# Ryan21wy/HSIMAE

Measured on AMD Instinct MI355X. Metric: HSI patches/sec (9x9x96, mask 75%) pretrain fwd+bwd, higher is better.
Workload: dtype bf16; 1 GPU; HSIMAE-Base pretrain fwd+bwd, 9x9x96 cubes, per-GPU batch 4096, mask 0.75, bf16 MFMA operands / fp32 accumulate + residual; per_gpu_batch=4096, global_batch=4096, parallelism=dp1

## Files before the change

hsimae_amd/build.py:

```python
from __future__ import annotations

import os
import subprocess
import sys
from concurrent.futures import ThreadPoolExecutor

HERE = os.path.dirname(os.path.abspath(__file__))
CSRC = os.path.join(HERE, "csrc")
LIB = os.path.join(HERE, "libhsimae_hip.so")
UNITS = ["gemm", "attn", "attn_wide", "wgrad", "elem", "pack", "fused_dec", "fused_enc", "loader", "scene", "gwpca", "api"]
HIPCC = os.environ.get("HIPCC", "/opt/rocm/bin/hipcc")
BASE_FLAGS = ["--offload-arch=gfx950", "-O3", "-fPIC", "-std=c++17", "-Wno-unused-value", "-fvisibility=hidden"]
FLAGS = BASE_FLAGS + os.environ.get("HSIMAE_HIPCC_EXTRA", "").split()


def flags_hash(flags: list[str]) -> str:
    import hashlib
    return hashlib.sha256(" ".join(flags).encode()).hexdigest()[:16]


def unit_flags(unit: str, flags: list[str]) -> list[str]:
    if unit != "api":
        return list(flags)
    return list(flags) + [f"-DHS_BUILD_FLAGS_HASH=0x{flags_hash(flags)}ULL", f"-DHS_BUILD_DEFAULT_FLAGS={int(flags == BASE_FLAGS)}",
                          f"-DHS_KERNEL_SOURCE_HASH=0x{kernel_source_hash()}ULL"]


def kernel_source_hash() -> str:
    import hashlib
    h = hashlib.sha256()
    files = sorted(os.path.join(CSRC, f) for f in os.listdir(CSRC) if f.endswith((".hip", ".h", ".cpp")))
    files.append(os.path.join(HERE, "..", "include", "hsimae_hip.h"))
    for f in files:
# ... 76 lines not shown
```

hsimae_amd/csrc/api.hip:

```cpp
#include "common.h"
#include "kernels.h"
#include "plan.h"
#include <vector>
#include <algorithm>
#include <cstring>
#include <cstdlib>
#include <mutex>
#include <unordered_map>
#include <initializer_list>

using namespace hsplan;

namespace {

#define CK(expr) do { int _e = (expr); if (_e) return _e; } while (0)
#define CK0(expr) do { int _e0 = (expr); if (_e0) return _e0; } while (0)

inline hipStream_t S(void* s) { return reinterpret_cast<hipStream_t>(s); }
struct BlkP {
    const float *n1w, *n1b, *bqkv, *pb, *n2w, *n2b, *w1b, *w3b, *w2b;
    const hs_bf16 *qkv, *p, *w1, *w3, *w2, *qkvT, *pT, *w13T, *w2T;
    const float *qf, *kf, *vf, *pf, *w1f, *w3f;
    int prec;
    struct I8 { const uint8_t* w; const uint8_t* s; } qkv8, p8, w1_8, w3_8, w2_8, qkvT8, pT8, w13T8, w2T8;
// ... 10 lines not shown
    const uint8_t* base8 = reinterpret_cast<const uint8_t*>(fbase + WL.f32_elems);
    auto i8 = [&](const Img8& im) { BlkP::I8 r; r.w = base8 + im.w; r.s = base8 + im.s; return r; };
    b.prec = HSIMAE_PREC_BF16;
    b.qkv8 = i8(w.qkv8); b.p8 = i8(w.p8); b.w1_8 = i8(w.w1_8); b.w3_8 = i8(w.w3_8); b.w2_8 = i8(w.w2_8);
    b.qkvT8 = i8(w.qkvT8); b.pT8 = i8(w.pT8); b.w13T8 = i8(w.w13T8); b.w2T8 = i8(w.w2T8);
    return b;
}
enum : uint32_t {
    SC_FUSED_DEC = 1u << 0,
    SC_DEC_SPLIT = 1u << 1,
    SC_FP8_UNFUSED = 1u << 2,
    SC_FUSED_MLP = 1u << 3,
    SC_ATTN_BLOCK = 1u << 4,
    SC_ATTN_BLOCK256 = 1u << 5,
    SC_ATTN_BLOCK_BWD = 1u << 6,
    SC_PROJ_BWD = 1u << 7,
    SC_LNBWD = 1u << 8,
    SC_LNBWD_512 = 1u << 9,
    SC_RECOMPUTE = 1u << 10,
    SC_WGRAD_SLAB = 1u << 11,
    SC_DEC_SLAB = 1u << 12,
    SC_PLANAR = 1u << 13,
    SC_ATTN_BLOCK256_BWD = 1u << 14,
};
uint32_t sched_from_env() {
    auto off = [](const char* name) { const char* e = getenv(name); return e && e[0] == '0'; };
    auto one = [](const char* name) { const char* e = getenv(name); return e && e[0] == '1'; };
    uint32_t b = 0;
    if (!off("HSIMAE_FUSED_DEC")) b |= SC_FUSED_DEC;
    if (!off("HSIMAE_DEC_SPLIT")) b |= SC_DEC_SPLIT;
    if (one("HSIMAE_FP8_UNFUSED")) b |= SC_FP8_UNFUSED;
    if (!off("HSIMAE_FUSED_MLP")) b |= SC_FUSED_MLP;
    if (!off("HSIMAE_FUSED_ATTN_BLOCK")) b |= SC_ATTN_BLOCK;
    if (!off("HSIMAE_FUSED_ATTN_BLOCK256")) b |= SC_ATTN_BLOCK256;
    if (!off("HSIMAE_FUSED_ATTN_BLOCK_BWD")) b |= SC_ATTN_BLOCK_BWD;
    if (!off("HSIMAE_FUSED_PROJ_BWD")) b |= SC_PROJ_BWD;
    if (!off("HSIMAE_FUSED_LNBWD")) b |= SC_LNBWD;
    if (!off("HSIMAE_FUSED_LNBWD_512")) b |= SC_LNBWD_512;
    if (!off("HSIMAE_ATTN_BWD_RECOMPUTE")) b |= SC_RECOMPUTE;
    if (!off("HSIMAE_WGRAD_SLAB")) b |= SC_WGRAD_SLAB;
    if (!off("HSIMAE_DEC_SLAB")) b |= SC_DEC_SLAB;
    if (!off("HSIMAE_WGRAD_PLANAR")) b |= SC_PLANAR;
    if (!off("HSIMAE_FUSED_ATTN_BLOCK256_BWD")) b |= SC_ATTN_BLOCK256_BWD;
    return b;
}
struct SchedRec { uint32_t enc = 0, dec = 0; bool has_enc = false, has_dec = false; uint64_t gen = 0; };
std::mutex g_sched_mu;
std::unordered_map<const void*, SchedRec> g_sched;
uint64_t g_sched_gen = 0;
void record_sched(const void* ws, bool enc, bool dec, uint32_t bits) {
    std::lock_guard<std::mutex> lk(g_sched_mu);
    if (g_sched.size() > 4096 && g_sched.find(ws) == g_sched.end()) {
        std::vector<uint64_t> gens;
        gens.reserve(g_sched.size());
        for (auto& kv : g_sched) gens.push_back(kv.second.gen);
        std::nth_element(gens.begin(), gens.begin() + gens.size() / 2, gens.end());
        const uint64_t cut = gens[gens.size() / 2];
        for (auto it = g_sched.begin(); it != g_sched.end();) it = it->second.gen < cut ? g_sched.erase(it) : std::next(it);
    }
    SchedRec& r = g_sched[ws];
    r.gen = ++g_sched_gen;
    if (enc) {
        r.enc = bits; r.has_enc = true;
        if (!dec) r.has_dec = false;
    }
    if (dec) { r.dec = bits; r.has_dec = true; }
// ... 151 lines not shown
    return HSIMAE_OK;
}


static bool wide_ln_fused(int d, int dp, bool f8, uint32_t sc) {
    return (sc & SC_LNBWD) && dp == d && (d == 256 || (d == 512 && f8 && (sc & SC_LNBWD_512)));
}

int block_bwd(const BlkP& P, uint32_t sc, const BlkOff& o, float* grads, const float* x_in, const BlkBuf& b, int64_t M, int d,
              int heads, int h, int hp, int Ts, int nsamples, int mode, int len_l, float* G0, const Scr& w,
              float* dx_out, int accumulate, hipStream_t s, int concurrent = 1, const float* rs_a = nullptr,
              const float* rs_m = nullptr, int64_t* det_acc = nullptr) {
    float* G1 = w.G1;
    GemmParams p = gp();
    const int dp = rup(d, 32);
    LnBwdParams l; std::memset(&l, 0, sizeof(l));
    l.M = (int)M; l.d = d; l.ld = dp; l.det_base = grads; l.det_acc = det_acc;
    const bool f8 = P.prec == HSIMAE_PREC_FP8;
    const bool f8u = f8 && (sc & SC_FP8_UNFUSED);
    auto w8 = [&](GemmParams& q, const BlkP::I8& a) { if (f8) { q.prec = HSIMAE_PREC_FP8; q.W8 = a.w; q.S8 = a.s; } };
    const bool fmlp = !f8u && fused_mlp_enabled(d, h, sc);
    bool g1b_done = false;
    const int hp64 = rup(hp, 64);
    const bool planar = fmlp && (sc & SC_PLANAR) && M % 32 == 0 && (M + kPlanePadRows) * 2 * (int64_t)(hp64 + 256) * 2 < (1ll << 32);
    const int prow = planar ? (int)M + HS_PLANE_PAD_ROWS : 0;
    if (fmlp) {
        CK(hs_enc_mlp_bwd(b.x1, G0, G1, b.u2, w.dh13, b.g, w.g0b, w.g1b, (int)M, d, mlp_ptrs(P, h), grads + o.n2w,
                          grads + o.n2b, s, rs_m, rs_a, HsDet{grads, reinterpret_cast<long long*>(det_acc)}, prow));
    } else {
        p.A = G0; p.lda = dp; p.M = (int)M; p.N = hp; p.K = dp; p.n_valid = hp; p.W = P.w2T; p.out = w.dh13; p.ldo = 2 * hp;
        p.h13 = b.h13; p.ldh = 2 * hp; p.hoff = hp; p.a_rowscale = rs_m;
        w8(p, P.w2T8);
        CK(hs_gemm(p, A_F32, E_SWIGLU_BWD, s));
        p = gp();
        p.A = w.dh13; p.lda = 2 * hp; p.M = (int)M; p.N = dp; p.K = 2 * hp; p.n_valid = d; p.W = P.w13T;
        w8(p, P.w13T8);
        if (wide_ln_fused(d, dp, f8, sc)) {
            p.out = G1; p.ldo = dp; p.res = G0; p.ldr = dp; p.lnx = b.x1; p.gamma = P.n2w; p.accumulate = 0;
            p.dgamma = grads + o.n2w; p.dbeta = grads + o.n2b; p.det_base = grads; p.det_acc = det_acc;
            if (!rs_a) { p.u_out = w.g1b; p.ldu = dp; g1b_done = true; }
            CK(hs_gemm(p, A_BF16, E_LN_BWD, s));
        } else {
            p.out = w.du; p.ldo = dp;
            CK(hs_gemm(p, A_BF16, E_F32, s));
            l.du = w.du; l.x = b.x1; l.gamma = P.n2w; l.dres = G0; l.dx = G1; l.accumulate = 0;
            l.dgamma = grads + o.n2w; l.dbeta = grads + o.n2b;
            CK(hs_ln_bwd(l, s));
        }
        CK(hs_rows_to_bf16(G0, w.g0b, M, dp, rs_m, s));
        if (!g1b_done) CK(hs_rows_to_bf16(G1, w.g1b, M, dp, rs_a, s));
    }
    auto run_wgrad = [&]() -> int {
        WgradParams g; std::memset(&g, 0, sizeof(g));
        auto task = [&](int, const void* dO, int ldo, const hs_bf16* A, int lda, int N, int K, int64_t dW, int64_t db) {
            WgradTask& t = g.t[g.ntasks++];
            t.dO = dO; t.dO_f32 = 0; t.ldo = ldo; t.A = A; t.lda = lda; t.N = N; t.K = K; t.dW = grads + dW; t.ldw = K;
            t.db = grads + db; t.dO_rowscale = nullptr;
        };
        task(0, w.dqkv, 3 * dp, b.u, dp, d, d, o.qw, o.qb);
        task(1, w.dqkv + dp, 3 * dp, b.u, dp, d, d, o.kw, o.kb);
        task(2, w.dqkv + 2 * dp, 3 * dp, b.u, dp, d, d, o.vw, o.vb);
        task(3, w.g1b, dp, b.o, dp, d, d, o.pw, o.pb);
        if (planar) {
            task(4, w.dh13, hp64, b.u2, dp, h, d, o.w1w, o.w1b); g.t[g.ntasks - 1].dO_plane_rows = prow;
            task(5, w.dh13 + (int64_t)hp64 * prow, hp64, b.u2, dp, h, d, o.w3w, o.w3b); g.t[g.ntasks - 1].dO_plane_rows = prow;
        } else {
            task(4, w.dh13, 2 * hp, b.u2, dp, h, d, o.w1w, o.w1b);
            task(5, w.dh13 + hp, 2 * hp, b.u2, dp, h, d, o.w3w, o.w3b);
        }
#ifdef HS_ABL_DW2
        if (!fmlp)
#endif
        { task(6, w.g0b, dp, b.g, planar ? hp64 : hp, d, h, o.w2w, o.w2b); g.t[g.ntasks - 1].A_plane_rows = prow; }
        g.M = (int)M; g.det_base = grads; g.det_acc = det_acc;
        g.slab = (sc & SC_WGRAD_SLAB) ? w.slab : nullptr;
        int tiles = 0;
        for (int i = 0; i < g.ntasks; ++i) tiles += ((g.t[i].N + 127) / 128) * ((g.t[i].K + 127) / 128);
        g.msplit = wgrad_msplit(tiles, M, concurrent);
        return hs_wgrad(g, s);
    };
    AttnParams a; std::memset(&a, 0, sizeof(a));
    a.qkv = b.qkv; a.ld = 3 * dp; a.d = d; a.heads = heads; a.hd = d / heads; a.Ts = Ts; a.nsamples = nsamples;
    a.mode = mode; a.len_l = len_l; a.o = b.o; a.ldo = dp; a.lse = b.lse; a.dout = w.dob; a.lddo = dp; a.dqkv = w.dqkv; a.kv_off = dp;
    const bool fuse_pb = (sc & SC_PROJ_BWD) != 0;
    const bool fuse_ln = (sc & SC_LNBWD) != 0;
    const bool rc = attn_bwd_recompute(d, dp, heads, h, Ts, f8u, sc);
    const bool blk_bwd = rc || (fuse_pb && fuse_ln && fmlp && !f8u && d == 128 && dp == d && hs_attn_proj_fusable(a) &&
                                (sc & SC_ATTN_BLOCK_BWD) && hs_attn_block_bwd_fusable(d, heads, Ts));
    const bool blk256_bwd = !blk_bwd && !f8 && dp == d && (sc & SC_ATTN_BLOCK256_BWD) && (sc & SC_LNBWD) && (sc & SC_PROJ_BWD) &&
                            hs_attn_block256_bwd_fusable(d, heads, Ts, nsamples);
    if (blk256_bwd) {
        CK(hs_attn_block256_bwd(b.qkv, b.lse, w.g1b, G1, x_in, P.n1w, P.pT, P.qkvT, w.dqkv, dx_out, grads + o.n1w, grads + o.n1b, grads,
                                reinterpret_cast<long long*>(det_acc), Ts, nsamples, mode, len_l, accumulate, s));
        CK(run_wgrad());
        return HSIMAE_OK;
    }
    if (blk_bwd) {
        CK(hs_attn_block_bwd(rc ? nullptr : b.qkv, b.u, P.qkv, P.bqkv, b.o, b.lse, w.g1b, G1, x_in, P.n1w, P.pT, P.qkvT, w.dqkv, dx_out,
                             grads + o.n1w, grads + o.n1b, grads, reinterpret_cast<long long*>(det_acc), Ts, nsamples, mode, len_l,
                             accumulate, s));
// ... 41 lines not shown
    if (!io) return HSIMAE_ENULL;
    c.N = io->N; c.len_t = io->len_t; c.len_l = io->len_l;
    if (c.N <= 0 || c.len_t < 1 || c.len_t > c.g.T || c.len_l < 1 || c.len_l > 9) return HSIMAE_EDIMS;
    c.K = c.len_t * c.len_l;
    c.Me = (int64_t)c.N * c.K; c.Md = (int64_t)c.N * c.g.TL;
    if (c.Md * 96 >= (1ll << 31) || c.Me * 3 * c.g.Dp >= (1ll << 31)) return HSIMAE_EUNSUPPORTED;
    make_playout(c.g, c.L);
    make_wlayout(c.g, c.W);
    if (need_ws) {
        if (!io->workspace || !io->params || !io->wpk) return HSIMAE_ENULL;
        if (reinterpret_cast<uintptr_t>(io->workspace) % 256) return HSIMAE_EALIGN;
        carve(c.g, c.N, c.K, reinterpret_cast<char*>(io->workspace), c.w);
        if (c.w.bytes > io->workspace_bytes) return HSIMAE_EDIMS;
    }
    return HSIMAE_OK;
}

}

extern "C" unsigned hs_variant_bits_gemm();
extern "C" unsigned hs_variant_bits_attn();
extern "C" unsigned hs_variant_bits_attn_wide();
extern "C" unsigned hs_variant_bits_wgrad();
extern "C" unsigned hs_variant_bits_elem();
extern "C" unsigned hs_variant_bits_pack();
extern "C" unsigned hs_variant_bits_fused_dec();
extern "C" unsigned hs_variant_bits_fused_enc();
extern "C" unsigned hs_variant_bits_loader();
extern "C" unsigned hs_variant_bits_scene();
extern "C" unsigned hs_variant_bits_gwpca();
#ifndef HS_KERNEL_SOURCE_HASH
#define HS_KERNEL_SOURCE_HASH 0ULL
#endif
#ifndef HS_BUILD_FLAGS_HASH
#define HS_BUILD_FLAGS_HASH 0ULL
#endif
#ifndef HS_BUILD_DEFAULT_FLAGS
#define HS_BUILD_DEFAULT_FLAGS 0
#endif

extern "C" {

int hsimae_version(void) { return HSIMAE_VERSION; }

int hsimae_build_info(hsimae_build_info_t* out) {
    if (!out) return HSIMAE_ENULL;
    out->abi_version = HSIMAE_VERSION;
    out->variant_bits = hs_variant_bits() | hs_variant_bits_gemm() | hs_variant_bits_attn() | hs_variant_bits_attn_wide() | hs_variant_bits_wgrad() | hs_variant_bits_elem() | hs_variant_bits_pack() | hs_variant_bits_fused_dec() | hs_variant_bits_fused_enc() | hs_variant_bits_loader() | hs_variant_bits_scene() | hs_variant_bits_gwpca();
    out->kernel_source_hash = HS_KERNEL_SOURCE_HASH;
    out->flags_hash = HS_BUILD_FLAGS_HASH;
    out->default_flags = HS_BUILD_DEFAULT_FLAGS;
    out->reserved = 0;
    return HSIMAE_OK;
}
const char* hsimae_variant_name(int bit) {
    switch (bit) {
#define HS_X(b, name) case b: return #name;
        HS_VARIANT_TABLE(HS_X)
#undef HS_X
        default: return nullptr;
    }
}

int hsimae_two_streams_active(void) { return side().ok ? 1 : 0; }
int hsimae_effective_precision(const hsimae_config* cfg) {
    if (!cfg) return HSIMAE_ENULL;
    Geo g; CK(make_geo(cfg, g));
    return (g.prec == HSIMAE_PREC_FP8 && (g.D >= 512 || (sched_from_env() & SC_FP8_UNFUSED))) ? HSIMAE_PREC_FP8 : HSIMAE_PREC_BF16;
}

const char* hsimae_strerror(int code) {
// ... 528 lines not shown
```

hsimae_amd/csrc/fused_enc.hip:

```cpp
#include "common.h"
#include "kernels.h"
#include <cstdlib>

#ifdef HS_PHASE_TIMING
__device__ unsigned long long hs_phase_cycles_enc[32];
extern "C" __attribute__((visibility("default"))) int hsimae_debug_phases_enc(unsigned long long* out, int reset) {
    int rc = (int)hipMemcpyFromSymbol(out, HIP_SYMBOL(hs_phase_cycles_enc), sizeof(unsigned long long) * 32);
    if (reset) { unsigned long long z[32] = {0}; rc |= (int)hipMemcpyToSymbol(HIP_SYMBOL(hs_phase_cycles_enc), z, sizeof(z)); }
    return rc;
}
#define PH_DECL unsigned long long ph_t0 = __builtin_readcyclecounter(), ph_acc[8] = {0, 0, 0, 0, 0, 0, 0, 0};
#define PH(i) { const unsigned long long ph_t = __builtin_readcyclecounter(); ph_acc[i] += ph_t - ph_t0; ph_t0 = ph_t; }
#define PH_FLUSH(base) if (threadIdx.x == 0) { for (int i = 0; i < 8; ++i) atomicAdd(&hs_phase_cycles_enc[(base) + i], ph_acc[i]); }
#else
#define PH_DECL
#define PH(i)
#define PH_FLUSH(base)
#endif

#ifndef HS_NT_A
#define HS_NT_A 1
#endif
#ifndef HS_NT_B
#define HS_NT_B 0
// ... 335 lines not shown
    HsDet det;
    int plane_rows;
};

__device__ __forceinline__ __amdgpu_buffer_rsrc_t panel_rsrc(const void* base, long long rows, int row_bytes) {
    const long long b = rows > 0 ? (rows < 4096 ? rows : 4096) * row_bytes : 0;
    return __builtin_amdgcn_make_buffer_rsrc(const_cast<void*>(base), 0, (int)b, 0x00020000);
}
__device__ __forceinline__ void bld8(__amdgpu_buffer_rsrc_t r, unsigned bo, float* o) {
    const f32x4 a = __builtin_bit_cast(f32x4, __builtin_amdgcn_raw_buffer_load_b128(r, (int)bo, 0, 0));
    const f32x4 b = __builtin_bit_cast(f32x4, __builtin_amdgcn_raw_buffer_load_b128(r, (int)bo + 16, 0, 0));
    o[0] = a[0]; o[1] = a[1]; o[2] = a[2]; o[3] = a[3]; o[4] = b[0]; o[5] = b[1]; o[6] = b[2]; o[7] = b[3];
}
typedef __attribute__((ext_vector_type(4))) unsigned int u32q;
__device__ __forceinline__ void bst8f(__amdgpu_buffer_rsrc_t r, unsigned bo, const float* v) {
    __builtin_amdgcn_raw_buffer_store_b128(__builtin_bit_cast(u32q, f32x4{v[0], v[1], v[2], v[3]}), r, (int)bo, 0, 0);
    __builtin_amdgcn_raw_buffer_store_b128(__builtin_bit_cast(u32q, f32x4{v[4], v[5], v[6], v[7]}), r, (int)bo + 16, 0, 0);
}
__device__ __forceinline__ void bst8h(__amdgpu_buffer_rsrc_t r, unsigned bo, bf16x8 v, int aux) {
    if (aux) __builtin_amdgcn_raw_buffer_store_b128(__builtin_bit_cast(u32q, v), r, (int)bo, 0, 2);
    else __builtin_amdgcn_raw_buffer_store_b128(__builtin_bit_cast(u32q, v), r, (int)bo, 0, 0);
}

template <int D, int HPE, bool LATE_ST = false>
__global__ __launch_bounds__(NTH, (MG<D, HPE>::WPC)) void enc_mlp_bwd_kernel(EncMlpBwdArgs p) {
    using G = MG<D, HPE>;
    constexpr int R = G::R;
    constexpr int LU = G::LU, LC = G::LC, LX = G::LX, NCH = G::NCH, KSD = G::KSD, KSH = G::KSH, LPR = G::LPR;
    extern __shared__ __attribute__((aligned(16))) char smem[];
    bf16_t* U2 = reinterpret_cast<bf16_t*>(smem);
    bf16_t* DYb = U2 + R * LU;
    bf16_t* DH1 = DYb + R * LU;
    bf16_t* DH3 = DH1 + R * LC;
    bf16_t* Gc = DH3 + R * LC;
    float* XS = reinterpret_cast<float*>(G::XS_AT_DY ? reinterpret_cast<char*>(DYb) : smem);
    const G8 q = geo8<D>();
    const int row0 = blockIdx.x * R;
    const EncMlpW& w = p.w;
    const int nt_h = HPE / 16;
    const int c8 = (threadIdx.x % LPR) * 8;
    constexpr bool late_stores = LATE_ST;

    PH_DECL
    constexpr int MT4 = R / 16, NJO = D / 64;
    FrN<KSD, 1> f1, f3, f2;
    f1.template load<false>(w.w1, KSD, q.wave, 0, nt_h, q.lane);
    f3.template load<false>(w.w3, KSD, q.wave, 0, nt_h, q.lane);
// ... 94 lines not shown
                    f1.template load<false>(w.w1, KSD, (c + 1) * 4 + q.wave, 0, nt_h, q.lane);
                    f3.template load<false>(w.w3, KSD, (c + 1) * 4 + q.wave, 0, nt_h, q.lane);
                    f2.template load<false>(w.w2T, KSD, (c + 1) * 4 + q.wave, 0, nt_h, q.lane);
                } else {
                    f1.load(w.w1, KSD, (c + 1) * 4 + q.wave, 0, nt_h, q.lane);
                    f3.load(w.w3, KSD, (c + 1) * 4 + q.wave, 0, nt_h, q.lane);
                    f2.load(w.w2T, KSD, (c + 1) * 4 + q.wave, 0, nt_h, q.lane);
                }
            }
#endif
#pragma unroll
            for (int mt = 0; mt < MT4; ++mt) {
                f32x4 gv, d1, d3;
#pragma unroll
                for (int r = 0; r < 4; ++r) {
                    const float a1 = h1[mt][r], a3 = h3[mt][r], dv = dg[mt][r];
                    const float sg = __builtin_amdgcn_rcpf(1.f + __expf(-a1));
                    const float sl = a1 * sg;
                    gv[r] = sl * a3;
                    d1[r] = dv * a3 * sg * (1.f + a1 * (1.f - sg));
                    d3[r] = dv * sl;
                }
                const int o = ctile<LC>(mt, q);
                *reinterpret_cast<bf16x4*>(Gc + o) = cvt4(gv);
                *reinterpret_cast<bf16x4*>(DH1 + o) = cvt4(d1);
                *reinterpret_cast<bf16x4*>(DH3 + o) = cvt4(d3);
            }
        }
        lds_barrier();
        PH(1)
        constexpr bool LATE = D >= 256;
        FrN<2, NJO> wa;
        FrN<1, NJO> wb0, wb1;
#ifdef HS_ABL_WSTREAM
        constexpr int cw = 0;
#else
        const int cw = c;
#endif
        wa.template load<false>(w.w13T, 2 * KSH, q.wave * NJO, 2 * cw, D / 16, q.lane);
        wb0.template load<false>(w.w13T, 2 * KSH, q.wave * NJO, KSH + 2 * cw, D / 16, q.lane);
        if constexpr (!LATE) wb1.template load<false>(w.w13T, 2 * KSH, q.wave * NJO, KSH + 2 * cw + 1, D / 16, q.lane);
        if (!late_stores && p.dh13) {
            const int ncol = (c * 64 + 64 <= HPE) ? 64 : HPE - c * 64;
            for (int pc = threadIdx.x; pc < R * 8; pc += NTH) {
                const int row = pc >> 3, k8 = (pc & 7) * 8;
                if (row0 + row < p.M && k8 < ncol) {
                    const size_t gr = (size_t)(row0 + row);
                    if (p.plane_rows) {
                        const size_t po = ((size_t)c * p.plane_rows + gr) * 64 + k8;
                        HS_NT(HS_NT_A, reinterpret_cast<bf16x8*>(p.g + po), *reinterpret_cast<const bf16x8*>(Gc + row * LC + (((k8 >> 3) ^ swzc<D>(row)) << 3)));
                        HS_NT(HS_NT_A, reinterpret_cast<bf16x8*>(p.dh13 + po), *reinterpret_cast<const bf16x8*>(DH1 + row * LC + (((k8 >> 3) ^ swzc<D>(row)) << 3)));
                        HS_NT(HS_NT_A, reinterpret_cast<bf16x8*>(p.dh13 + (size_t)NCH * 64 * p.plane_rows + po), *reinterpret_cast<const bf16x8*>(DH3 + row * LC + (((k8 >> 3) ^ swzc<D>(row)) << 3)));
                        continue;
                    }
#ifndef HS_ABL_DW2
                    HS_NT(HS_NT_A, reinterpret_cast<bf16x8*>(p.g + gr * HPE + c * 64 + k8), *reinterpret_cast<const bf16x8*>(Gc + row * LC + (((k8 >> 3) ^ swzc<D>(row)) << 3)));
#endif
                    HS_NT(HS_NT_A, reinterpret_cast<bf16x8*>(p.dh13 + gr * 2 * HPE + c * 64 + k8), *reinterpret_cast<const bf16x8*>(DH1 + row * LC + (((k8 >> 3) ^ swzc<D>(row)) << 3)));
                    HS_NT(HS_NT_A, reinterpret_cast<bf16x8*>(p.dh13 + gr * 2 * HPE + HPE + c * 64 + k8), *reinterpret_cast<const bf16x8*>(DH3 + row * LC + (((k8 >> 3) ^ swzc<D>(row)) << 3)));
                }
            }
        }
        PH(2)
        constexpr bool kHalfLast = (HPE % 64) != 0;
#pragma unroll
        for (int ks = 0; ks < 2; ++ks) {
            if (kHalfLast && c == NCH - 1 && ks == 1) continue;
            if constexpr (LATE) {
                if (ks == 0 && !(kHalfLast && c == NCH - 1)) wb1.template load<false>(w.w13T, 2 * KSH, q.wave * NJO, KSH + 2 * cw + 1, D / 16, q.lane);
            }
#pragma unroll
            for (int mt = 0; mt < MT4; ++mt) {
                const bf16x8 a1 = cfrag<LC>(DH1, mt, ks, q);
                const bf16x8 a3 = cfrag<LC>(DH3, mt, ks, q);
#pragma unroll
                for (int j = 0; j < NJO; ++j) {
                    du2[mt][j] = mfma16(wa.b[ks][j], a1, du2[mt][j]);
                    du2[mt][j] = mfma16(ks == 0 ? wb0.b[0][j] : wb1.b[0][j], a3, du2[mt][j]);
                }
            }
        }
        if (late_stores && p.dh13) {
            const int ncol = (c * 64 + 64 <= HPE) ? 64 : HPE - c * 64;
            const unsigned plane = (unsigned)p.plane_rows * 64u * 2u;
            const __amdgpu_buffer_rsrc_t rg = __builtin_amdgcn_make_buffer_rsrc(p.g, 0, (int)(NCH * plane), 0x00020000);
            const __amdgpu_buffer_rsrc_t rd = __builtin_amdgcn_make_buffer_rsrc(p.dh13, 0, (int)(2 * NCH * plane), 0x00020000);
            typedef __attribute__((ext_vector_type(4))) unsigned int u4;
            int tid = threadIdx.x;
            asm volatile("" : "+v"(tid));
#pragma unroll
            for (int it = 0; it < (R * 8 + NTH - 1) / NTH; ++it) {
                const int pc = tid + it * NTH, row = pc >> 3, k8 = (pc & 7) * 8;
                const bool ok = pc < R * 8 && row0 + row < p.M && k8 < ncol;
                const int lrow = ok ? row : 0;
                const int lo = lrow * LC + (((k8 >> 3) ^ swzc<D>(lrow)) << 3);
                const unsigned po = ok ? (unsigned)c * plane + ((unsigned)(row0 + row) * 64u + (unsigned)k8) * 2u : 0xffffff00u;
                __builtin_amdgcn_raw_buffer_store_b128(__builtin_bit_cast(u4, *reinterpret_cast<const bf16x8*>(Gc + lo)), rg, (int)po, 0, HS_NT_A ? 2 : 0);
                __builtin_amdgcn_raw_buffer_store_b128(__builtin_bit_cast(u4, *reinterpret_cast<const bf16x8*>(DH1 + lo)), rd, (int)po, 0, HS_NT_A ? 2 : 0);
                __builtin_amdgcn_raw_buffer_store_b128(__builtin_bit_cast(u4, *reinterpret_cast<const bf16x8*>(DH3 + lo)), rd, (int)(ok ? po + NCH * plane : po), 0, HS_NT_A ? 2 : 0);
            }
        }
        lds_barrier();
        PH(3)
    }
#pragma unroll
// ... 72 lines not shown

}

static int hp_of(int hidden) { return (hidden + 31) / 32 * 32; }

bool hs_enc_mlp_fused_supported(int d, int hidden) {
    return (d == 128 && hp_of(hidden) == 352) || (d == 256 && hp_of(hidden) == 704) || (d == 64 && hp_of(hidden) == 192);
}

static EncMlpW mkw(const EncMlpPtrs& b) {
    EncMlpW w;
    w.n2w = b.n2w; w.n2b = b.n2b; w.w1b = b.w1b; w.w3b = b.w3b; w.w2b = b.w2b;
    w.w1 = b.w1; w.w3 = b.w3; w.w2 = b.w2; w.w2T = b.w2T; w.w13T = b.w13T; w.h = b.h;
    return w;
}

template <int D, int HP>
static void set_attrs() {
    static bool done = false;
    if (done) return;
    (void)hipFuncSetAttribute(reinterpret_cast<const void*>(enc_mlp_fwd_kernel<D, HP>), hipFuncAttributeMaxDynamicSharedMemorySize, MG<D, HP>::LDS_FWD);
    (void)hipFuncSetAttribute(reinterpret_cast<const void*>(enc_mlp_bwd_kernel<D, HP, false>), hipFuncAttributeMaxDynamicSharedMemorySize, MG<D, HP>::LDS_BWD);
    (void)hipFuncSetAttribute(reinterpret_cast<const void*>(enc_mlp_bwd_kernel<D, HP, true>), hipFuncAttributeMaxDynamicSharedMemorySize, MG<D, HP>::LDS_BWD);
    done = true;
}

template <int D, int HP>
static int fwd_grid(int M) {
    const int panels = (M + MG<D, HP>::R - 1) / MG<D, HP>::R;
    if (!MG<D, HP>::PERSIST) return panels;
    static int slots = 0;
    if (!slots) slots = 256 * MG<D, HP>::WPCF;
    return panels < slots ? panels : slots;
}

static int launch_fwd(const EncMlpFwdArgs& a, int M, int d, hipStream_t s) {
    if (d == 128) {
        set_attrs<128, 352>();
        hipLaunchKernelGGL((enc_mlp_fwd_kernel<128, 352>), dim3(fwd_grid<128, 352>(M)), dim3(NTH), (MG<128, 352>::LDS_FWD), s, a);
    } else if (d == 256) {
        set_attrs<256, 704>();
        hipLaunchKernelGGL((enc_mlp_fwd_kernel<256, 704>), dim3(fwd_grid<256, 704>(M)), dim3(NTH), (MG<256, 704>::LDS_FWD), s, a);
    } else if (d == 64) {
        set_attrs<64, 192>();
        hipLaunchKernelGGL((enc_mlp_fwd_kernel<64, 192>), dim3(fwd_grid<64, 192>(M)), dim3(NTH), (MG<64, 192>::LDS_FWD), s, a);
    } else {
        return HS_EUNSUPPORTED;
    }
    return (int)hipGetLastError();
}

int hs_enc_mlp_fwd(const float* x1, const float* res2, float* x2, int M, int d, const EncMlpPtrs& b, hipStream_t s,
                   const float* rowscale) {
    if (M <= 0) return HS_OK;
    EncMlpFwdArgs a;
    a.x1 = x1; a.res2 = res2; a.x2 = x2; a.M = M; a.w = mkw(b); a.rowscale = rowscale;
    return launch_fwd(a, M, d, s);
}

template <int D, int HP>
static void launch_bwd_t(const EncMlpBwdArgs& a, int M, hipStream_t s) {
    constexpr int R = MG<D, HP>::R;
    set_attrs<D, HP>();
    const bool late = HS_MLPB_LATE_STORES && D >= 256 && a.dh13 && a.plane_rows > 0 && (size_t)2 * MG<D, HP>::NCH * a.plane_rows * 128 < 0xffffff00u;
    if (late) hipLaunchKernelGGL((enc_mlp_bwd_kernel<D, HP, true>), dim3((M + R - 1) / R), dim3(NTH), (MG<D, HP>::LDS_BWD), s, a);
    else hipLaunchKernelGGL((enc_mlp_bwd_kernel<D, HP, false>), dim3((M + R - 1) / R), dim3(NTH), (MG<D, HP>::LDS_BWD), s, a);
}

static int launch_bwd(const EncMlpBwdArgs& a, int M, int d, hipStream_t s) {
    if (d == 128) launch_bwd_t<128, 352>(a, M, s);
    else if (d == 256) launch_bwd_t<256, 704>(a, M, s);
    else if (d == 64) launch_bwd_t<64, 192>(a, M, s);
    else return HS_EUNSUPPORTED;
    return (int)hipGetLastError();
}

static EncMlpBwdArgs mk_bwd(const float* x1, const float* dy, float* dx1, hs_bf16* u2, hs_bf16* dh13, hs_bf16* g, hs_bf16* dyb,
                            hs_bf16* dx1b, int M, const EncMlpPtrs& b, float* g_n2w, float* g_n2b, const float* rs_mlp,
                            const float* rs_attn, HsDet det, int plane_rows) {
    EncMlpBwdArgs a; a.x1 = x1; a.dy = dy; a.dx1 = dx1; a.u2 = u2; a.dh13 = dh13; a.g = g; a.M = M; a.w = mkw(b);
    a.g_n2w = g_n2w; a.g_n2b = g_n2b; a.dyb = dyb; a.dx1b = dx1b; a.rs_mlp = rs_mlp; a.rs_attn = rs_attn; a.det = det;
    a.plane_rows = plane_rows;
    return a;
}

int hs_enc_mlp_bwd(const float* x1, const float* dy, float* dx1, hs_bf16* u2, hs_bf16* dh13, hs_bf16* g, hs_bf16* dyb,
                   hs_bf16* dx1b, int M, int d, const EncMlpPtrs& b, float* g_n2w, float* g_n2b, hipStream_t s,
// ... 7 lines not shown
```

hsimae_amd/csrc/kernels.h:

```cpp
#pragma once
#include "common.h"
#include "../../include/hsimae_hip.h"

enum AKind { A_BF16 = HSIMAE_A_BF16, A_F32 = HSIMAE_A_F32, A_F32_LN = HSIMAE_A_F32_LN };
enum Epi { E_BF16 = HSIMAE_E_BF16, E_F32 = HSIMAE_E_F32, E_RES_F32 = HSIMAE_E_RES_F32,
           E_POS_F32 = HSIMAE_E_POS_F32, E_SWIGLU = HSIMAE_E_SWIGLU, E_SWIGLU_BWD = HSIMAE_E_SWIGLU_BWD,
           E_LN_BWD = HSIMAE_E_LN_BWD };

typedef hsimae_gemm_params GemmParams;
typedef hsimae_pack_desc PackDesc;
typedef hsimae_attn_params AttnParams;
typedef hsimae_wgrad_task WgradTask;
typedef hsimae_wgrad_params WgradParams;
typedef hsimae_lnbwd_params LnBwdParams;
typedef hsimae_mask_params MaskParams;
typedef hsimae_patch_params PatchParams;
typedef hsimae_assemble_params AssembleParams;
typedef hsimae_loss_params LossParams;
typedef hsimae_cube_params CubeParams;
typedef hsimae_scene_params SceneParams;

int hs_gemm(const GemmParams& p, int akind, int epi, hipStream_t s);
int hs_gemm_tiled(const GemmParams& p, int akind, int epi, int bm, int kc, hipStream_t s);
int hs_pack(const PackDesc* descs_dev, int ndesc, int max_elems, hipStream_t s);
// ... 52 lines not shown
int hs_attn_block_bwd(const hs_bf16* qkv, const hs_bf16* u, const hs_bf16* wqkv, const float* bqkv, const hs_bf16* o, const float* lse,
                      const hs_bf16* dx1b, const float* dx1, const float* x, const float* gamma, const hs_bf16* wpT, const hs_bf16* wqkvT,
                      hs_bf16* dqkv, float* dx, float* dgamma, float* dbeta, const float* det_base, long long* det_acc, int Ts,
                      int nsamples, int mode, int len_l, int accumulate, hipStream_t s);
int hs_attn_block_fwd(const float* x, const float* n1w, const float* n1b, const hs_bf16* wqkv, const float* bqkv, const hs_bf16* wp,
                      const float* pb, hs_bf16* u, hs_bf16* qkv, hs_bf16* o, float* lse, float* x1, const float* rowscale, int Ts,
                      int nsamples, int mode, int len_l, hipStream_t s);
bool hs_attn_block256_fusable(int d, int heads, int Ts, int nsamples);
int hs_attn_block256_fwd(const float* x, const float* n1w, const float* n1b, const hs_bf16* wqkv, const float* bqkv, const hs_bf16* wp,
                         const float* pb, hs_bf16* u, hs_bf16* qkv, hs_bf16* o, float* lse, float* x1, const float* rowscale, int Ts,
                         int nsamples, int mode, int len_l, hipStream_t s);
bool hs_attn_block256_bwd_fusable(int d, int heads, int Ts, int nsamples);
int hs_attn_block256_bwd(const hs_bf16* qkv, const float* lse, const hs_bf16* dx1b, const float* dx1, const float* x, const float* gamma,
                         const hs_bf16* wpT, const hs_bf16* wqkvT, hs_bf16* dqkv, float* dx, float* dgamma, float* dbeta,
                         const float* det_base, long long* det_acc, int Ts, int nsamples, int mode, int len_l, int accumulate,
                         hipStream_t s);
bool hs_enc_mlp_fused_supported(int d, int hidden);
int hs_enc_mlp_fwd(const float* x1, const float* res2, float* x2, int M, int d, const EncMlpPtrs& b, hipStream_t s,
                   const float* rowscale = nullptr);
int hs_enc_mlp_bwd(const float* x1, const float* dy, float* dx1, hs_bf16* u2, hs_bf16* dh13, hs_bf16* g, hs_bf16* dyb,
                   hs_bf16* dx1b, int M, int d, const EncMlpPtrs& b, float* g_n2w, float* g_n2b, hipStream_t s,
                   const float* rs_mlp = nullptr, const float* rs_attn = nullptr, HsDet det = HsDet{nullptr, nullptr}, int plane_rows = 0);

int hs_adamw(float* p, const float* g, float* m, float* v, const unsigned char* group, int64_t n, float lr, float b1, float b2,
             float eps, float wd, int step, hipStream_t s);
```

Before: 257,300 patches/s.

## Add fused MLP weight-gradient kernel that recomputes activations instead of storing dh13/g

Adds a new wgrad_mlp kernel for d=128 encoder MLP backward. It recomputes h1/h3 and the gate gradients on the fly from u2 and dy and accumulates dW1, dW3, dW2 and the biases directly. The existing MLP backward kernel gets a NO_OPS variant that skips writing the dh13 and g intermediates, and the generic wgrad tasks 4-6 are dropped. This is meant to remove the global-memory round trip of the large hidden-dimension intermediates. The cost is redundant forward GEMMs inside the wgrad kernel, and deterministic accumulation is routed through a hs_gadd path.

Result: slower. 239,500 patches/s (-6.9%).

```diff
diff --git a/hsimae_amd/build.py b/hsimae_amd/build.py
--- a/hsimae_amd/build.py
+++ b/hsimae_amd/build.py
@@ -8,7 +8,7 @@
 HERE = os.path.dirname(os.path.abspath(__file__))
 CSRC = os.path.join(HERE, "csrc")
 LIB = os.path.join(HERE, "libhsimae_hip.so")
-UNITS = ["gemm", "attn", "attn_wide", "wgrad", "elem", "pack", "fused_dec", "fused_enc", "loader", "scene", "gwpca", "api"]
+UNITS = ["gemm", "attn", "attn_wide", "wgrad", "wgrad_mlp", "elem", "pack", "fused_dec", "fused_enc", "loader", "scene", "gwpca", "api"]
 HIPCC = os.environ.get("HIPCC", "/opt/rocm/bin/hipcc")
 BASE_FLAGS = ["--offload-arch=gfx950", "-O3", "-fPIC", "-std=c++17", "-Wno-unused-value", "-fvisibility=hidden"]
 FLAGS = BASE_FLAGS + os.environ.get("HSIMAE_HIPCC_EXTRA", "").split()
diff --git a/hsimae_amd/csrc/api.hip b/hsimae_amd/csrc/api.hip
--- a/hsimae_amd/csrc/api.hip
+++ b/hsimae_amd/csrc/api.hip
@@ -56,6 +56,7 @@
     SC_DEC_SLAB = 1u << 12,
     SC_PLANAR = 1u << 13,
     SC_ATTN_BLOCK256_BWD = 1u << 14,
+    SC_WGRAD_MLP = 1u << 15,
 };
 uint32_t sched_from_env() {
     auto off = [](const char* name) { const char* e = getenv(name); return e && e[0] == '0'; };
@@ -76,6 +77,7 @@
     if (!off("HSIMAE_DEC_SLAB")) b |= SC_DEC_SLAB;
     if (!off("HSIMAE_WGRAD_PLANAR")) b |= SC_PLANAR;
     if (!off("HSIMAE_FUSED_ATTN_BLOCK256_BWD")) b |= SC_ATTN_BLOCK256_BWD;
+    if (!off("HSIMAE_WGRAD_MLP")) b |= SC_WGRAD_MLP;
     return b;
 }
 struct SchedRec { uint32_t enc = 0, dec = 0; bool has_enc = false, has_dec = false; uint64_t gen = 0; };
@@ -273,11 +275,15 @@
     const bool fmlp = !f8u && fused_mlp_enabled(d, h, sc);
     bool g1b_done = false;
     const int hp64 = rup(hp, 64);
-    const bool planar = fmlp && (sc & SC_PLANAR) && M % 32 == 0 && (M + kPlanePadRows) * 2 * (int64_t)(hp64 + 256) * 2 < (1ll << 32);
+    const bool wmlp = fmlp && !f8 && (sc & SC_WGRAD_MLP) && d == 128 && dp == d && hs_wgrad_mlp_supported(d, h);
+    const bool planar = fmlp && !wmlp && (sc & SC_PLANAR) && M % 32 == 0 && (M + kPlanePadRows) * 2 * (int64_t)(hp64 + 256) * 2 < (1ll << 32);
     const int prow = planar ? (int)M + HS_PLANE_PAD_ROWS : 0;
     if (fmlp) {
-        CK(hs_enc_mlp_bwd(b.x1, G0, G1, b.u2, w.dh13, b.g, w.g0b, w.g1b, (int)M, d, mlp_ptrs(P, h), grads + o.n2w,
-                          grads + o.n2b, s, rs_m, rs_a, HsDet{grads, reinterpret_cast<long long*>(det_acc)}, prow));
+        CK(hs_enc_mlp_bwd(b.x1, G0, G1, b.u2, wmlp ? nullptr : w.dh13, wmlp ? nullptr : b.g, w.g0b, w.g1b, (int)M, d, mlp_ptrs(P, h),
+                          grads + o.n2w, grads + o.n2b, s, rs_m, rs_a, HsDet{grads, reinterpret_cast<long long*>(det_acc)}, prow));
+        if (wmlp)
+            CK(hs_wgrad_mlp(b.u2, w.g0b, (int)M, d, mlp_ptrs(P, h), grads + o.w1w, grads + o.w3w, grads + o.w2w, grads + o.w1b,
+                            grads + o.w3b, grads + o.w2b, HsDet{grads, reinterpret_cast<long long*>(det_acc)}, s));
     } else {
         p.A = G0; p.lda = dp; p.M = (int)M; p.N = hp; p.K = dp; p.n_valid = hp; p.W = P.w2T; p.out = w.dh13; p.ldo = 2 * hp;
         p.h13 = b.h13; p.ldh = 2 * hp; p.hoff = hp; p.a_rowscale = rs_m;
@@ -312,7 +318,8 @@
         task(1, w.dqkv + dp, 3 * dp, b.u, dp, d, d, o.kw, o.kb);
         task(2, w.dqkv + 2 * dp, 3 * dp, b.u, dp, d, d, o.vw, o.vb);
         task(3, w.g1b, dp, b.o, dp, d, d, o.pw, o.pb);
-        if (planar) {
+        if (wmlp) {
+        } else if (planar) {
             task(4, w.dh13, hp64, b.u2, dp, h, d, o.w1w, o.w1b); g.t[g.ntasks - 1].dO_plane_rows = prow;
             task(5, w.dh13 + (int64_t)hp64 * prow, hp64, b.u2, dp, h, d, o.w3w, o.w3b); g.t[g.ntasks - 1].dO_plane_rows = prow;
         } else {
@@ -322,11 +329,12 @@
 #ifdef HS_ABL_DW2
         if (!fmlp)
 #endif
-        { task(6, w.g0b, dp, b.g, planar ? hp64 : hp, d, h, o.w2w, o.w2b); g.t[g.ntasks - 1].A_plane_rows = prow; }
+        if (!wmlp) { task(6, w.g0b, dp, b.g, planar ? hp64 : hp, d, h, o.w2w, o.w2b); g.t[g.ntasks - 1].A_plane_rows = prow; }
         g.M = (int)M; g.det_base = grads; g.det_acc = det_acc;
         g.slab = (sc & SC_WGRAD_SLAB) ? w.slab : nullptr;
         int tiles = 0;
         for (int i = 0; i < g.ntasks; ++i) tiles += ((g.t[i].N + 127) / 128) * ((g.t[i].K + 127) / 128);
+        if (wmlp && det_acc) tiles += 3 * ((h + 127) / 128) * ((d + 127) / 128);
         g.msplit = wgrad_msplit(tiles, M, concurrent);
         return hs_wgrad(g, s);
     };
@@ -414,6 +422,7 @@
 extern "C" unsigned hs_variant_bits_attn();
 extern "C" unsigned hs_variant_bits_attn_wide();
 extern "C" unsigned hs_variant_bits_wgrad();
+extern "C" unsigned hs_variant_bits_wgrad_mlp();
 extern "C" unsigned hs_variant_bits_elem();
 extern "C" unsigned hs_variant_bits_pack();
 extern "C" unsigned hs_variant_bits_fused_dec();
@@ -438,7 +447,7 @@
 int hsimae_build_info(hsimae_build_info_t* out) {
     if (!out) return HSIMAE_ENULL;
     out->abi_version = HSIMAE_VERSION;
-    out->variant_bits = hs_variant_bits() | hs_variant_bits_gemm() | hs_variant_bits_attn() | hs_variant_bits_attn_wide() | hs_variant_bits_wgrad() | hs_variant_bits_elem() | hs_variant_bits_pack() | hs_variant_bits_fused_dec() | hs_variant_bits_fused_enc() | hs_variant_bits_loader() | hs_variant_bits_scene() | hs_variant_bits_gwpca();
+    out->variant_bits = hs_variant_bits() | hs_variant_bits_gemm() | hs_variant_bits_attn() | hs_variant_bits_attn_wide() | hs_variant_bits_wgrad() | hs_variant_bits_wgrad_mlp() | hs_variant_bits_elem() | hs_variant_bits_pack() | hs_variant_bits_fused_dec() | hs_variant_bits_fused_enc() | hs_variant_bits_loader() | hs_variant_bits_scene() | hs_variant_bits_gwpca();
     out->kernel_source_hash = HS_KERNEL_SOURCE_HASH;
     out->flags_hash = HS_BUILD_FLAGS_HASH;
     out->default_flags = HS_BUILD_DEFAULT_FLAGS;
diff --git a/hsimae_amd/csrc/fused_enc.hip b/hsimae_amd/csrc/fused_enc.hip
--- a/hsimae_amd/csrc/fused_enc.hip
+++ b/hsimae_amd/csrc/fused_enc.hip
@@ -381,7 +381,7 @@
     else __builtin_amdgcn_raw_buffer_store_b128(__builtin_bit_cast(u32q, v), r, (int)bo, 0, 0);
 }
 
-template <int D, int HPE, bool LATE_ST = false>
+template <int D, int HPE, bool LATE_ST = false, bool NO_OPS = false>
 __global__ __launch_bounds__(NTH, (MG<D, HPE>::WPC)) void enc_mlp_bwd_kernel(EncMlpBwdArgs p) {
     using G = MG<D, HPE>;
     constexpr int R = G::R;
@@ -522,7 +522,7 @@
                     d3[r] = dv * sl;
                 }
                 const int o = ctile<LC>(mt, q);
-                *reinterpret_cast<bf16x4*>(Gc + o) = cvt4(gv);
+                if constexpr (!NO_OPS) *reinterpret_cast<bf16x4*>(Gc + o) = cvt4(gv);
                 *reinterpret_cast<bf16x4*>(DH1 + o) = cvt4(d1);
                 *reinterpret_cast<bf16x4*>(DH3 + o) = cvt4(d3);
             }
@@ -540,7 +540,7 @@
         wa.template load<false>(w.w13T, 2 * KSH, q.wave * NJO, 2 * cw, D / 16, q.lane);
         wb0.template load<false>(w.w13T, 2 * KSH, q.wave * NJO, KSH + 2 * cw, D / 16, q.lane);
         if constexpr (!LATE) wb1.template load<false>(w.w13T, 2 * KSH, q.wave * NJO, KSH + 2 * cw + 1, D / 16, q.lane);
-        if (!late_stores && p.dh13) {
+        if constexpr (!NO_OPS) if (!late_stores && p.dh13) {
             const int ncol = (c * 64 + 64 <= HPE) ? 64 : HPE - c * 64;
             for (int pc = threadIdx.x; pc < R * 8; pc += NTH) {
                 const int row = pc >> 3, k8 = (pc & 7) * 8;
@@ -580,7 +580,7 @@
                 }
             }
         }
-        if (late_stores && p.dh13) {
+        if constexpr (!NO_OPS) if (late_stores && p.dh13) {
             const int ncol = (c * 64 + 64 <= HPE) ? 64 : HPE - c * 64;
             const unsigned plane = (unsigned)p.plane_rows * 64u * 2u;
             const __amdgpu_buffer_rsrc_t rg = __builtin_amdgcn_make_buffer_rsrc(p.g, 0, (int)(NCH * plane), 0x00020000);
@@ -699,6 +699,8 @@
     (void)hipFuncSetAttribute(reinterpret_cast<const void*>(enc_mlp_fwd_kernel<D, HP>), hipFuncAttributeMaxDynamicSharedMemorySize, MG<D, HP>::LDS_FWD);
     (void)hipFuncSetAttribute(reinterpret_cast<const void*>(enc_mlp_bwd_kernel<D, HP, false>), hipFuncAttributeMaxDynamicSharedMemorySize, MG<D, HP>::LDS_BWD);
     (void)hipFuncSetAttribute(reinterpret_cast<const void*>(enc_mlp_bwd_kernel<D, HP, true>), hipFuncAttributeMaxDynamicSharedMemorySize, MG<D, HP>::LDS_BWD);
+    if constexpr (D == 128)
+        (void)hipFuncSetAttribute(reinterpret_cast<const void*>(enc_mlp_bwd_kernel<D, HP, false, true>), hipFuncAttributeMaxDynamicSharedMemorySize, MG<D, HP>::LDS_BWD);
     done = true;
 }
 
@@ -740,6 +742,12 @@
     constexpr int R = MG<D, HP>::R;
     set_attrs<D, HP>();
     const bool late = HS_MLPB_LATE_STORES && D >= 256 && a.dh13 && a.plane_rows > 0 && (size_t)2 * MG<D, HP>::NCH * a.plane_rows * 128 < 0xffffff00u;
+    if constexpr (D == 128) {
+        if (!a.dh13 && !a.g) {
+            hipLaunchKernelGGL((enc_mlp_bwd_kernel<D, HP, false, true>), dim3((M + R - 1) / R), dim3(NTH), (MG<D, HP>::LDS_BWD), s, a);
+            return;
+        }
+    }
     if (late) hipLaunchKernelGGL((enc_mlp_bwd_kernel<D, HP, true>), dim3((M + R - 1) / R), dim3(NTH), (MG<D, HP>::LDS_BWD), s, a);
     else hipLaunchKernelGGL((enc_mlp_bwd_kernel<D, HP, false>), dim3((M + R - 1) / R), dim3(NTH), (MG<D, HP>::LDS_BWD), s, a);
 }
diff --git a/hsimae_amd/csrc/kernels.h b/hsimae_amd/csrc/kernels.h
--- a/hsimae_amd/csrc/kernels.h
+++ b/hsimae_amd/csrc/kernels.h
@@ -98,5 +98,9 @@
                    hs_bf16* dx1b, int M, int d, const EncMlpPtrs& b, float* g_n2w, float* g_n2b, hipStream_t s,
                    const float* rs_mlp = nullptr, const float* rs_attn = nullptr, HsDet det = HsDet{nullptr, nullptr}, int plane_rows = 0);
 
+bool hs_wgrad_mlp_supported(int d, int hidden);
+int hs_wgrad_mlp(const hs_bf16* u2, const hs_bf16* dyb, int M, int d, const EncMlpPtrs& b, float* dW1, float* dW3, float* dW2,
+                 float* db1, float* db3, float* db2, HsDet det, hipStream_t s);
+
 int hs_adamw(float* p, const float* g, float* m, float* v, const unsigned char* group, int64_t n, float lr, float b1, float b2,
              float eps, float wd, int step, hipStream_t s);
diff --git a/hsimae_amd/csrc/wgrad_mlp.hip b/hsimae_amd/csrc/wgrad_mlp.hip
--- /dev/null
+++ b/hsimae_amd/csrc/wgrad_mlp.hip
@@ -0,0 +1,237 @@
+#include "common.h"
+#include "kernels.h"
+#include <algorithm>
+
+namespace {
+
+constexpr int WD = 128;
+constexpr int RS = 64;
+constexpr int NTHR = 512;
+constexpr int LT = WD + 16;
+constexpr int LI = 64 + 16;
+constexpr int TILE = RS * LT, IMG = RS * LI;
+constexpr int LDS_BYTES = (4 * TILE + 3 * IMG) * 2;
+
+struct WgradMlpArgs {
+    const bf16_t *u2, *dyb;
+    const bf16_t *w1, *w3, *w2T;
+    const float *w1b, *w3b;
+    float *dW1, *dW3, *dW2, *db1, *db3, *db2;
+    int M, h, nt_h, nch, msplit;
+    HsDet det;
+};
+
+typedef __attribute__((address_space(3))) bf16x4* lds_b64_ptr;
+
+template <int LD>
+__device__ __forceinline__ bf16x8 frag_tr(const bf16_t* tile, int mbase, int col0, int lane) {
+    const int g = lane >> 4, q = (lane & 15) >> 2, pq = lane & 3;
+    const bf16_t* a0 = tile + (mbase + 4 * g + q) * LD + col0 + 4 * pq;
+    const bf16x4 lo = __builtin_amdgcn_ds_read_tr16_b64_v4bf16((lds_b64_ptr)(a0));
+    const bf16x4 hi = __builtin_amdgcn_ds_read_tr16_b64_v4bf16((lds_b64_ptr)(a0 + 16 * LD));
+    return __builtin_shufflevector(lo, hi, 0, 1, 2, 3, 4, 5, 6, 7);
+}
+
+__device__ __forceinline__ bf16x4 cvt4(f32x4 v) {
+    bf16x4 r;
+    r[0] = (bf16_t)v[0]; r[1] = (bf16_t)v[1]; r[2] = (bf16_t)v[2]; r[3] = (bf16_t)v[3];
+    return r;
+}
+
+__global__ __launch_bounds__(NTHR) void wgrad_mlp_kernel(WgradMlpArgs p) {
+    extern __shared__ __attribute__((aligned(16))) char smem[];
+    bf16_t* T = reinterpret_cast<bf16_t*>(smem);
+    bf16_t* DH1 = T + 4 * TILE;
+    bf16_t* DH3 = DH1 + IMG;
+    bf16_t* Gc = DH3 + IMG;
+    const int tid = threadIdx.x, lane = tid & 63, wave = __builtin_amdgcn_readfirstlane(tid >> 6);
+    const int c16 = lane & 15, g = lane >> 4;
+
+    const int xcd = blockIdx.x & 7, li = blockIdx.x >> 3;
+    const int c = li % p.nch, ms = xcd + 8 * (li / p.nch);
+    if (ms >= p.msplit) return;
+    const int nsteps = (p.M + RS - 1) / RS;
+    const int spw = (nsteps + p.msplit - 1) / p.msplit;
+    const int sbeg = ms * spw, send = min(nsteps, sbeg + spw);
+    if (sbeg >= send) return;
+
+    const int wn = wave & 3, wm = wave >> 2;
+    const int nt = c * 4 + wn;
+    bf16x8 f1[4], f3[4], f2[4];
+#pragma unroll
+    for (int ks = 0; ks < 4; ++ks) {
+        f1[ks] = zero8(); f3[ks] = zero8(); f2[ks] = zero8();
+        if (nt < p.nt_h) {
+            const size_t o = ((size_t)(nt * 4 + ks) * 64 + lane) * 8;
+            f1[ks] = *reinterpret_cast<const bf16x8*>(p.w1 + o);
+            f3[ks] = *reinterpret_cast<const bf16x8*>(p.w3 + o);
+            f2[ks] = *reinterpret_cast<const bf16x8*>(p.w2T + o);
+        }
+    }
+    f32x4 b1, b3;
+#pragma unroll
+    for (int r = 0; r < 4; ++r) {
+        const int col = nt * 16 + g * 4 + r;
+        b1[r] = col < p.h ? p.w1b[col] : 0.f;
+        b3[r] = col < p.h ? p.w3b[col] : 0.f;
+    }
+
+    const int lr = tid >> 4, c8 = (tid & 15) * 8;
+    bf16x8 ru[2], rd[2];
+    auto load_rows = [&](int step) {
+#pragma unroll
+        for (int i = 0; i < 2; ++i) {
+            const int row = step * RS + lr + 32 * i;
+            ru[i] = zero8(); rd[i] = zero8();
+            if (row < p.M) {
+                ru[i] = *reinterpret_cast<const bf16x8*>(p.u2 + (size_t)row * WD + c8);
+                rd[i] = *reinterpret_cast<const bf16x8*>(p.dyb + (size_t)row * WD + c8);
+            }
+        }
+    };
+    float bs2[8];
+#pragma unroll
+    for (int e = 0; e < 8; ++e) bs2[e] = 0.f;
+    auto store_rows = [&](int stage) {
+        bf16_t* U = T + stage * 2 * TILE;
+#pragma unroll
+        for (int i = 0; i < 2; ++i) {
+            *reinterpret_cast<bf16x8*>(U + (lr + 32 * i) * LT + c8) = ru[i];
+            *reinterpret_cast<bf16x8*>(U + TILE + (lr + 32 * i) * LT + c8) = rd[i];
+            if (c == 0) {
+#pragma unroll
+                for (int e = 0; e < 8; ++e) bs2[e] += bf2f(rd[i][e]);
+            }
+        }
+    };
+
+    const int ht = wn, dq = wm;
+    f32x4 acc[3][4];
+#pragma unroll
+    for (int i = 0; i < 3; ++i)
+#pragma unroll
+        for (int j = 0; j < 4; ++j) acc[i][j] = f32x4{0.f, 0.f, 0.f, 0.f};
+    f32x4 bs1 = {0.f, 0.f, 0.f, 0.f}, bs3 = {0.f, 0.f, 0.f, 0.f};
+
+    load_rows(sbeg);
+    store_rows(0);
+    if (sbeg + 1 < send) load_rows(sbeg + 1);
+    for (int s = sbeg; s < send; ++s) {
+        const int st = (s - sbeg) & 1;
+        const bf16_t* U = T + st * 2 * TILE;
+        const bf16_t* DY = U + TILE;
+        lds_barrier();
+        {
+            f32x4 h1[2], h3[2], dg[2];
+#pragma unroll
+            for (int mt = 0; mt < 2; ++mt) { h1[mt] = b1; h3[mt] = b3; dg[mt] = f32x4{0.f, 0.f, 0.f, 0.f}; }
+#pragma unroll
+            for (int ks = 0; ks < 4; ++ks)
+#pragma unroll
+                for (int mt = 0; mt < 2; ++mt) {
+                    const int o = ((2 * wm + mt) * 16 + c16) * LT + ks * 32 + 8 * g;
+                    const bf16x8 au = *reinterpret_cast<const bf16x8*>(U + o);
+                    const bf16x8 ad = *reinterpret_cast<const bf16x8*>(DY + o);
+                    h1[mt] = mfma16(f1[ks], au, h1[mt]);
+                    h3[mt] = mfma16(f3[ks], au, h3[mt]);
+                    dg[mt] = mfma16(f2[ks], ad, dg[mt]);
+                }
+#pragma unroll
+            for (int mt = 0; mt < 2; ++mt) {
+                f32x4 gv, d1, d3;
+#pragma unroll
+                for (int r = 0; r < 4; ++r) {
+                    const float a1 = h1[mt][r], a3 = h3[mt][r], dv = dg[mt][r];
+                    const float sg = __builtin_amdgcn_rcpf(1.f + __expf(-a1));
+                    const float sl = a1 * sg;
+                    gv[r] = sl * a3;
+                    d1[r] = dv * a3 * sg * (1.f + a1 * (1.f - sg));
+                    d3[r] = dv * sl;
+                }
+                const bf16x4 q1 = cvt4(d1), q3 = cvt4(d3);
+#pragma unroll
+                for (int r = 0; r < 4; ++r) { bs1[r] += bf2f(q1[r]); bs3[r] += bf2f(q3[r]); }
+                const int o = ((2 * wm + mt) * 16 + c16) * LI + wn * 16 + 4 * g;
+                *reinterpret_cast<bf16x4*>(Gc + o) = cvt4(gv);
+                *reinterpret_cast<bf16x4*>(DH1 + o) = q1;
+                *reinterpret_cast<bf16x4*>(DH3 + o) = q3;
+            }
+        }
+        if (s + 1 < send) {
+            store_rows(st ^ 1);
+            if (s + 2 < send) load_rows(s + 2);
+        }
+        lds_barrier();
+#pragma unroll
+        for (int kk = 0; kk < RS / 32; ++kk) {
+            const bf16x8 a1 = frag_tr<LI>(DH1, kk * 32, ht * 16, lane);
+            const bf16x8 a3 = frag_tr<LI>(DH3, kk * 32, ht * 16, lane);
+            const bf16x8 ag = frag_tr<LI>(Gc, kk * 32, ht * 16, lane);
+#pragma unroll
+            for (int j = 0; j < 4; ++j) {
+                const bf16x8 bu = frag_tr<LT>(U, kk * 32, (dq * 4 + j) * 16, lane);
+                const bf16x8 bd = frag_tr<LT>(DY, kk * 32, (dq * 4 + j) * 16, lane);
+                acc[0][j] = mfma16(a1, bu, acc[0][j]);
+                acc[1][j] = mfma16(a3, bu, acc[1][j]);
+                acc[2][j] = mfma16(ag, bd, acc[2][j]);
+            }
+        }
+    }
+
+#pragma unroll
+    for (int j = 0; j < 4; ++j)
+#pragma unroll
+        for (int r = 0; r < 4; ++r) {
+            const int hid = c * 64 + ht * 16 + g * 4 + r;
+            const int col = (dq * 4 + j) * 16 + c16;
+            if (hid < p.h) {
+                hs_gadd(p.det, p.dW1 + (size_t)hid * WD + col, acc[0][j][r]);
+                hs_gadd(p.det, p.dW3 + (size_t)hid * WD + col, acc[1][j][r]);
+                hs_gadd(p.det, p.dW2 + (size_t)col * p.h + hid, acc[2][j][r]);
+            }
+        }
+#pragma unroll
+    for (int r = 0; r < 4; ++r) {
+        const float s1 = lanes_sum<16>(bs1[r]), s3 = lanes_sum<16>(bs3[r]);
+        const int hid = nt * 16 + g * 4 + r;
+        if (c16 == 0 && hid < p.h) { hs_gadd(p.det, p.db1 + hid, s1); hs_gadd(p.det, p.db3 + hid, s3); }
+    }
+    if (c == 0) {
+#pragma unroll
+        for (int e = 0; e < 8; ++e) {
+            const float s2 = rows_sum(bs2[e]);
+            if (g == 0) hs_gadd(p.det, p.db2 + c8 + e, s2);
+        }
+    }
+}
+
+}
+
+bool hs_wgrad_mlp_supported(int d, int hidden) { return d == WD && hidden >= 1; }
+
+int hs_wgrad_mlp(const hs_bf16* u2, const hs_bf16* dyb, int M, int d, const EncMlpPtrs& b, float* dW1, float* dW3, float* dW2,
+                 float* db1, float* db3, float* db2, HsDet det, hipStream_t s) {
+    if (M <= 0) return HS_OK;
+    if (!hs_wgrad_mlp_supported(d, b.h)) return HS_EUNSUPPORTED;
+    if (!u2 || !dyb || !dW1 || !dW3 || !dW2 || !db1 || !db3 || !db2) return HS_ENULL;
+    if ((reinterpret_cast<uintptr_t>(u2) | reinterpret_cast<uintptr_t>(dyb)) & 15) return HS_EALIGN;
+    static bool attrs = false;
+    if (!attrs) {
+        attrs = true;
+        (void)hipFuncSetAttribute(reinterpret_cast<const void*>(wgrad_mlp_kernel), hipFuncAttributeMaxDynamicSharedMemorySize, LDS_BYTES);
+    }
+    WgradMlpArgs a;
+    a.u2 = u2; a.dyb = dyb; a.w1 = b.w1; a.w3 = b.w3; a.w2T = b.w2T; a.w1b = b.w1b; a.w3b = b.w3b;
+    a.dW1 = dW1; a.dW3 = dW3; a.dW2 = dW2; a.db1 = db1; a.db3 = db3; a.db2 = db2;
+    a.M = M; a.h = b.h;
+    const int hp = (b.h + 31) / 32 * 32;
+    a.nt_h = hp / 16; a.nch = (hp + 63) / 64;
+    const int nsteps = (M + RS - 1) / RS;
+    a.msplit = std::max(1, std::min(8 * std::max(1, 32 / a.nch), nsteps));
+    a.det = det;
+    const dim3 grid(8 * a.nch * ((a.msplit + 7) / 8));
+    hipLaunchKernelGGL(wgrad_mlp_kernel, grid, dim3(NTHR), LDS_BYTES, s, a);
+    return (int)hipGetLastError();
+}
+
+HS_UNIT_VARIANT_BITS(wgrad_mlp)
```
